# yahoo0742/COSNet

Measured on AMD Instinct MI355X. Metric: frame-pairs/sec (fwd+bwd) at 473x473 RGBD, higher is better.
Workload: dtype bf16; 1 GPU; RGBDSegmentation_RAA train step (fwd+loss+bwd+SGD), 473x473, batch 4 pairs/GPU; model=RGBDSegmentation_RAA(Bottleneck,[3,4,23,3],[3,4,6,3],1), global_batch=4, parallelism=dp1

## Files before the change

### cosnet_amd/csrc/gemm.hip

```cpp
#include "common.h"
#include "gemm.h"
#include "gemm_dev.h"
#include "../../include/cosnet_hip.h"

#include <type_traits>

namespace {

template <class T> struct Frag;
template <> struct Frag<bf16> { typedef bf16x8 type; };
template <> struct Frag<float> { typedef f32x4 type; };

__device__ __forceinline__ int mc_swz(int k, int granules_per_row) {
  int h = (k & 3) | (((k >> 3) & 1) << 2);
  return (granules_per_row >= 32 ? h : (h & 3)) << 2;
}

__device__ __forceinline__ int mc_swz8(int k) { return (k & 7) ^ ((k >> 5) & 1); }

__device__ __attribute__((aligned(16))) unsigned g_zero16[4];

__device__ __forceinline__ void glds16(const void* src, char* lds_wave_base) {
  __builtin_amdgcn_global_load_lds((const __attribute__((address_space(1))) void*)src,
                                   (__attribute__((address_space(3))) void*)lds_wave_base, 16, 0, 0);
// ... 726 lines not shown
          else if (p.wt)
            __builtin_amdgcn_raw_buffer_store_b128(pk, crs, (int)(((long long)(row - m0) * p.ldc + col) * 2), 0, 16);
          else
            *(u32x4*)dst = pk;
          if (smode) Chunk<bf16>::unpack(pk, v);
        } else {
          if (cmode == 2) {
            f32x4 q0 = *(const f32x4*)dst, q1 = *(const f32x4*)(dst + 4);
#pragma unroll
            for (int e = 0; e < 4; ++e) { v[e] += q0[e]; v[4 + e] += q1[e]; }
          }
          if (p.wt == 4) {
            __builtin_nontemporal_store(*(f32x4*)&v[0], (f32x4*)dst);
            __builtin_nontemporal_store(*(f32x4*)&v[4], (f32x4*)(dst + 4));
          } else if (p.wt) {
            const int off = (int)(((long long)(row - m0) * p.ldc + col) * 4);
            __builtin_amdgcn_raw_buffer_store_b128(__builtin_bit_cast(u32x4, *(f32x4*)&v[0]), crs, off, 0, 16);
            __builtin_amdgcn_raw_buffer_store_b128(__builtin_bit_cast(u32x4, *(f32x4*)&v[4]), crs, off + 16, 0, 16);
          } else {
            *(f32x4*)dst = *(f32x4*)&v[0];
            *(f32x4*)(dst + 4) = *(f32x4*)&v[4];
          }
        }
      } else {
#pragma unroll
        for (int e = 0; e < 8; ++e)
          if (col + e < p.N) {
            store_c<CT>(dst + e, v[e], cmode);
            v[e] = tof((CT)v[e]);
          }
      }
#ifndef CN_EPI_NOACC
      if constexpr (smode == 1) {
        const bool inA = row < segA_end;
#pragma unroll
        for (int e = 0; e < 8; ++e) {
          const float d = (col + e < p.N) ? v[e] - sk[e] : 0.f;
          if (inA) { sa1[e] += d; sa2[e] = fmaf(d, d, sa2[e]); }
          else { sb1[e] += d; sb2[e] = fmaf(d, d, sb2[e]); }
        }
      } else if constexpr (smode == 2) {
        float xv[8];
        if (full) {
          if constexpr (sizeof(CT) == 2) Chunk<bf16>::unpack(xpf[it], xv);
          else { *(u32x4*)&xv[0] = xpf[2 * it]; *(u32x4*)&xv[4] = xpf[2 * it + 1]; }
        } else {
          const CT* xs = (const CT*)p.br_x + (long long)row * p.br_ldx + col;
#pragma unroll
          for (int e = 0; e < 8; ++e) xv[e] = (col + e < p.N) ? tof(xs[e]) : 0.f;
        }
#pragma unroll
        for (int e = 0; e < 8; ++e) {
          float dd = (col + e < p.N && fmaf(xv[e], bk1[e], bsf[e]) > 0.f) ? v[e] : 0.f;
          sa1[e] += dd;
          sa2[e] = fmaf(dd, xv[e] - bmu[e], sa2[e]);
        }
      }
#endif
    }
    __syncthreads();
  }
#ifdef CN_EPI_NORED
  if constexpr (false) {
#else
  if constexpr (smode != 0) {
#endif
    constexpr int NW = NT / 64;
    const int nq = smode == 1 ? 4 : 2;
#pragma unroll
    for (int e = 0; e < 8; ++e) {
#pragma unroll
      for (int o = GPR; o < 64; o <<= 1) {
        sa1[e] += __shfl_xor(sa1[e], o, 64);
        sa2[e] += __shfl_xor(sa2[e], o, 64);
        if (smode == 1) {
          sb1[e] += __shfl_xor(sb1[e], o, 64);
          sb2[e] += __shfl_xor(sb2[e], o, 64);
        }
      }
    }
    float* red = cs;
    if (lane < GPR) {
#pragma unroll
      for (int e = 0; e < 8; ++e) {
        red[(wave * 4 + 0) * BN + c0t + e] = sa1[e];
        red[(wave * 4 + 1) * BN + c0t + e] = sa2[e];
        red[(wave * 4 + 2) * BN + c0t + e] = sb1[e];
        red[(wave * 4 + 3) * BN + c0t + e] = sb2[e];
      }
    }
    __syncthreads();
    float* ws = ((p.ngroup && p.grp.ST[batch]) ? p.grp.ST[batch] : p.st_ws) + (long long)tm * p.N;
    for (int t = tid; t < nq * BN; t += NT) {
      const int q = t / BN, c = t % BN;
      float a = 0.f;
#pragma unroll
      for (int w = 0; w < NW; ++w) a += red[(w * 4 + q) * BN + c];
      if (smode == 2 && q == 1 && n0 + c < p.N) a *= p.br_invstd[n0 + c];
      if (n0 + c < p.N) ws[(long long)(smode == 1 ? q + 1 : q) * p.st_plane + n0 + c] = a;
    }
    if (smode == 1 && tid < GPR) {
#pragma unroll
      for (int e = 0; e < 8; ++e)
        if (n0 + c0t + e < p.N) ws[n0 + c0t + e] = sk[e];
    }
  }
}

struct TileCfg { int bm, bn, wm, wn, s, pp; };
static constexpr TileCfg kCfg[] = {
    {128, 64, 2, 2, 2},
    {128, 128, 2, 2, 2},
    {128, 128, 2, 2, 3},
    {256, 128, 4, 2, 3},
    {128, 256, 2, 4, 3},
    {256, 256, 2, 4, 2},
    {128, 64, 2, 2, 4},
    {128, 128, 2, 2, 4},
    {256, 128, 4, 2, 2},
    {128, 256, 2, 4, 2},
    {256, 256, 4, 2, 2},
    {128, 128, 4, 2, 2},
    {128, 64, 4, 2, 2},
    {128, 128, 4, 2, 3},
    {128, 128, 4, 2, 4},
    {256, 128, 4, 2, 3},
    {128, 64, 4, 2, 4},
    {64, 128, 2, 4, 2},
    {256, 128, 4, 2, 3, 1},
    {128, 256, 2, 4, 3, 1},
    {256, 256, 2, 4, 2, 1},
};
constexpr int kNumCfg = sizeof(kCfg) / sizeof(kCfg[0]);
static int g_force_cfg = -1;

static long long cfg_blocks(int c, const GemmArgs& a, int batch) {
  return (long long)((a.M + kCfg[c].bm - 1) / kCfg[c].bm) * ((a.N + kCfg[c].bn - 1) / kCfg[c].bn) *
         batch * a.nsplit;
}

static long long tiles_of(int c, int M, int N) {
  return (long long)((M + kCfg[c].bm - 1) / kCfg[c].bm) * ((N + kCfg[c].bn - 1) / kCfg[c].bn);
}
static int heuristic_cfg(int M, int N, int K, int bz) {
  if (N <= 64) return 12;
  if (N >= 512 && K >= 2048 && tiles_of(10, M, N) * bz >= 200) return 20;
  if (tiles_of(11, M, N) * bz <= 256 && K >= 512) return 13;
  if (N >= 1024 && K <= 512 && tiles_of(10, M, N) * bz >= 200) return 10;
  return 11;
}

static int pick_cfg(const GemmArgs& a, int batch) {
  if (g_force_cfg >= 0 && g_force_cfg < kNumCfg) return g_force_cfg;
  if (a.cfg >= 0 && a.cfg < kNumCfg) return a.cfg;
  return heuristic_cfg(a.M, a.N, a.K, batch * a.nsplit);
}

template <class T, class CT, int C, int LA, int LB, int EPI = 0>
static int launch_c(const GemmArgs& a, int batch, hipStream_t st) {
  constexpr TileCfg c = kCfg[C];
  dim3 grid((a.M + c.bm - 1) / c.bm, (a.N + c.bn - 1) / c.bn, batch * a.nsplit);
  hipLaunchKernelGGL((gemm_kernel<T, CT, c.bm, c.bn, c.wm, c.wn, c.s, LA, LB, EPI, c.pp>), grid,
                     dim3(c.wm * c.wn * 64), 0, st, a);
  CN_CHECK_LAUNCH();
  return 0;
}

template <class T, int LA, int EPI>
static int launch_epi(const GemmArgs& a, int batch, hipStream_t st) {
  if constexpr (sizeof(T) == 4) {
    if (a.N <= 64 || cfg_blocks(1, a, batch) < 384) return launch_c<T, T, 0, LA, L_KC_DENSE, EPI>(a, batch, st);
    return launch_c<T, T, 1, LA, L_KC_DENSE, EPI>(a, batch, st);
  } else {
    switch (pick_cfg(a, batch)) {
      case 10: return launch_c<T, T, 10, LA, L_KC_DENSE, EPI>(a, batch, st);
      case 11: return launch_c<T, T, 11, LA, L_KC_DENSE, EPI>(a, batch, st);
      case 12: return launch_c<T, T, 12, LA, L_KC_DENSE, EPI>(a, batch, st);
      case 13: return launch_c<T, T, 13, LA, L_KC_DENSE, EPI>(a, batch, st);
      case 18: return launch_c<T, T, 18, LA, L_KC_DENSE, EPI>(a, batch, st);
      case 19: return launch_c<T, T, 19, LA, L_KC_DENSE, EPI>(a, batch, st);
      case 20: return launch_c<T, T, 20, LA, L_KC_DENSE, EPI>(a, batch, st);
      default: return CN_ERR_UNSUPPORTED;
    }
  }
}


template <class T, class CT, int LA, int LB>
static int launch_tile(const GemmArgs& a, int batch, hipStream_t st) {
  if constexpr (sizeof(T) == 2 && sizeof(CT) == 2 && (LA == L_KC_DENSE || LA == L_KC_CONV) &&
                LB == L_KC_DENSE) {
    if (a.c_mode == 2 && !a.row_map && !a.ngroup) {
      switch (pick_cfg(a, batch)) {
        case 10: return launch_c<T, CT, 10, LA, LB, 3>(a, batch, st);
        case 11: return launch_c<T, CT, 11, LA, LB, 3>(a, batch, st);
        case 12: return launch_c<T, CT, 12, LA, LB, 3>(a, batch, st);
        case 13: return launch_c<T, CT, 13, LA, LB, 3>(a, batch, st);
        case 20: return launch_c<T, CT, 20, LA, LB, 3>(a, batch, st);
        default: break;
      }
    }
  }
  if constexpr (sizeof(T) == 4) {
    if (a.N <= 64 || cfg_blocks(1, a, batch) < 384) return launch_c<T, CT, 0, LA, LB>(a, batch, st);
    return launch_c<T, CT, 1, LA, LB>(a, batch, st);
  } else {
    switch (pick_cfg(a, batch)) {
      case 0: return launch_c<T, CT, 0, LA, LB>(a, batch, st);
      case 1: return launch_c<T, CT, 1, LA, LB>(a, batch, st);
      case 2: return launch_c<T, CT, 2, LA, LB>(a, batch, st);
      case 3: return launch_c<T, CT, 3, LA, LB>(a, batch, st);
      case 4: return launch_c<T, CT, 4, LA, LB>(a, batch, st);
      case 5: return launch_c<T, CT, 5, LA, LB>(a, batch, st);
      case 6: return launch_c<T, CT, 6, LA, LB>(a, batch, st);
      case 7: return launch_c<T, CT, 7, LA, LB>(a, batch, st);
      case 8: return launch_c<T, CT, 8, LA, LB>(a, batch, st);
      case 9: return launch_c<T, CT, 9, LA, LB>(a, batch, st);
      case 10: return launch_c<T, CT, 10, LA, LB>(a, batch, st);
      case 11: return launch_c<T, CT, 11, LA, LB>(a, batch, st);
      case 13: return launch_c<T, CT, 13, LA, LB>(a, batch, st);
      case 14: return launch_c<T, CT, 14, LA, LB>(a, batch, st);
      case 15: return launch_c<T, CT, 15, LA, LB>(a, batch, st);
      case 16: return launch_c<T, CT, 16, LA, LB>(a, batch, st);
      case 17: return launch_c<T, CT, 17, LA, LB>(a, batch, st);
      case 18: case 19: case 20: {
        constexpr bool kc = LA != L_MC_DENSE && LA != L_MC_CONV && LB != L_MC_DENSE && LB != L_MC_CONV;
        if constexpr (kc) {
          const int c = pick_cfg(a, batch);
          if (c == 18) return launch_c<T, CT, 18, LA, LB>(a, batch, st);
          if (c == 19) return launch_c<T, CT, 19, LA, LB>(a, batch, st);
          return launch_c<T, CT, 20, LA, LB>(a, batch, st);
        } else {
          if (pick_cfg(a, batch) == 20) return launch_c<T, CT, 10, LA, LB>(a, batch, st);
          return launch_c<T, CT, 11, LA, LB>(a, batch, st);
        }
      }
      default: return launch_c<T, CT, 12, LA, LB>(a, batch, st);
    }
  }
}

template <class T, class CT>
static int launch_conv_g(const GemmArgs& a, int batch, hipStream_t st) {
  if constexpr (sizeof(T) == 4) {
    if (a.N <= 64 || cfg_blocks(1, a, batch) < 384) return launch_c<T, CT, 0, L_KC_CONV_G, L_KC_DENSE>(a, batch, st);
    return launch_c<T, CT, 1, L_KC_CONV_G, L_KC_DENSE>(a, batch, st);
  } else {
    const int c = pick_cfg(a, batch);
    if (c == 12) return launch_c<T, CT, 12, L_KC_CONV_G, L_KC_DENSE>(a, batch, st);
    if (c == 13) return launch_c<T, CT, 13, L_KC_CONV_G, L_KC_DENSE>(a, batch, st);
    return launch_c<T, CT, 11, L_KC_CONV_G, L_KC_DENSE>(a, batch, st);
  }
}

template <class T, class CT>
static int launch_kinds(const GemmArgs& a, int la, int lb, int batch, hipStream_t st) {
#define CN_CASE(A_, B_) \
  if (la == A_ && lb == B_) return launch_tile<T, CT, A_, B_>(a, batch, st);
  if (la == L_KC_CONV_G && lb == L_KC_DENSE) return launch_conv_g<T, CT>(a, batch, st);
  CN_CASE(L_KC_DENSE, L_KC_DENSE)
  CN_CASE(L_KC_CONV, L_KC_DENSE)
  CN_CASE(L_KC_DENSE, L_MC_DENSE)
  CN_CASE(L_MC_DENSE, L_MC_DENSE)
  CN_CASE(L_MC_DENSE, L_MC_CONV)
#undef CN_CASE
  return -10;
}

template <class CT, int LA, class T8 = f8e4m3>
static int launch_f8(const GemmArgs& a, int batch, hipStream_t st) {
  const int c = pick_cfg(a, batch);
  if constexpr (sizeof(CT) == 2 && std::is_same<T8, f8e4m3>::value) {
    if (a.st_mode == 1) {
      if (c == 12) return launch_c<T8, CT, 12, LA, L_KC_DENSE, 1>(a, batch, st);
      if (c == 13) return launch_c<T8, CT, 13, LA, L_KC_DENSE, 1>(a, batch, st);
      return launch_c<T8, CT, 11, LA, L_KC_DENSE, 1>(a, batch, st);
    }
  }
  if (a.st_mode) return CN_ERR_UNSUPPORTED;
  if (c == 12) return launch_c<T8, CT, 12, LA, L_KC_DENSE>(a, batch, st);
  if (c == 13) return launch_c<T8, CT, 13, LA, L_KC_DENSE>(a, batch, st);
  return launch_c<T8, CT, 11, LA, L_KC_DENSE>(a, batch, st);
}

template <int LB>
static int launch_f8_mc(const GemmArgs& a, int batch, hipStream_t st) {
  if (a.cfg == 13) return launch_c<f8e5m2, float, 13, L_MC_DENSE, LB>(a, batch, st);
  return launch_c<f8e5m2, float, 11, L_MC_DENSE, LB>(a, batch, st);
}

static bool buf_ok(int kind, const GemmArgs& a, bool is_a, int esz) {
  const long long ld = is_a ? a.lda : a.ldb;
  const ConvGeom& g = is_a ? a.ga : a.gb;
  const long long kspan = a.nsplit > 1 ? a.k_chunk : a.K;
  if (kind == L_KC_DENSE) return 256 * ld * esz < 0x80000000ll && (long long)a.K * esz < 0xFFFF0000ll;
  if (kind == L_KC_CONV) return (long long)g.N * g.H * g.W * ld * esz < 0x80000000ll;
  if (kind == L_MC_DENSE) return (kspan + 128) * ld * esz < 0xFFFF0000ll && 128 * ld * esz < 0x80000000ll;
  return true;
}

static int g_ws_mode = 1;
static size_t g_ws_launches = 0;
static bool ws_heuristic(const GemmArgs& a) {
  return a.K <= 256 && a.N >= 4 * a.K && a.M >= 8192;
}
static bool ws_eligible(const GemmArgs& a, int dtype, int c_f32, int la, int lb, int batch) {
  if (!g_ws_mode || g_force_cfg >= 0 || a.cfg >= 0) return false;
  if (dtype != DT_BF16 || c_f32 || la != L_KC_DENSE || lb != L_KC_DENSE) return false;
  if (batch != 1 || a.nsplit != 1 || a.row_map || a.ngroup || a.st_mode) return false;
  if ((a.c_mode != 0 && a.c_mode != 2) || a.bias || a.alpha != 1.f || a.scale_a || a.scale_b) return false;
  if (!cn_gemm_ws_supports(a)) return false;
  return g_ws_mode >= 2 || ws_heuristic(a);
}

int cn_gemm_dispatch(const GemmArgs& a_in, int dtype, int c_f32, int la, int lb, int batch, hipStream_t st) {
  GemmArgs a = a_in;
  a.wt = a.c_mode != 1 && a.c_mode != 3 ? 4 : 0;
  if (a.M <= 0 || a.N <= 0 || batch <= 0) return 0;
  const int esz = (dtype == DT_FP8 || dtype == DT_FP8_E5M2) ? 1 : dtype == DT_BF16 ? 2 : 4;
  const int bk = 128 / esz;
  if (la == L_KC_CONV && (a.ga.C % bk != 0 || !buf_ok(L_KC_CONV, a, true, esz))) la = L_KC_CONV_G;
  if (!buf_ok(la, a, true, esz) || !buf_ok(lb, a, false, esz)) return CN_ERR_SHAPE;
  if (ws_eligible(a, dtype, c_f32, la, lb, batch)) {
    ++g_ws_launches;
    return cn_gemm_ws_launch(a, g_ws_mode == 3 ? 1 : 0, st);
  }
  if (dtype == DT_FP8) {
    if (lb != L_KC_DENSE || a.nsplit != 1) return CN_ERR_UNSUPPORTED;
    if (a.st_mode && (a.st_mode != 1 || batch != 1 || a.row_map || a.c_mode || c_f32)) return CN_ERR_UNSUPPORTED;
    if (la == L_KC_DENSE) return c_f32 ? launch_f8<float, L_KC_DENSE>(a, batch, st) : launch_f8<bf16, L_KC_DENSE>(a, batch, st);
    if (la == L_KC_CONV) return c_f32 ? launch_f8<float, L_KC_CONV>(a, batch, st) : launch_f8<bf16, L_KC_CONV>(a, batch, st);
    if (la == L_KC_CONV_G) return c_f32 ? launch_f8<float, L_KC_CONV_G>(a, batch, st) : launch_f8<bf16, L_KC_CONV_G>(a, batch, st);
    return CN_ERR_UNSUPPORTED;
  }
  if (dtype == DT_FP8_E5M2 && la == L_MC_DENSE) {
    if (!c_f32 || a.st_mode || a.row_map || a.c_mode == 1 || a.c_mode == 2) return CN_ERR_UNSUPPORTED;
    if (lb == L_MC_DENSE) return launch_f8_mc<L_MC_DENSE>(a, batch, st);
    if (lb == L_MC_CONV) return launch_f8_mc<L_MC_CONV>(a, batch, st);
    return CN_ERR_UNSUPPORTED;
  }
  if (dtype == DT_FP8_E5M2) {
    if (lb != L_KC_DENSE || a.st_mode || a.nsplit != 1 || c_f32) return CN_ERR_UNSUPPORTED;
    if (la == L_KC_DENSE) return launch_f8<bf16, L_KC_DENSE, f8e5m2>(a, batch, st);
    if (la == L_KC_CONV) return launch_f8<bf16, L_KC_CONV, f8e5m2>(a, batch, st);
    if (la == L_KC_CONV_G) return launch_f8<bf16, L_KC_CONV_G, f8e5m2>(a, batch, st);
    return CN_ERR_UNSUPPORTED;
  }
  if (a.st_mode) {
    if ((batch != 1 && !(a.ngroup == batch && a.st_mode == 1)) || a.nsplit != 1 || a.row_map || a.c_mode ||
        lb != L_KC_DENSE || (la != L_KC_DENSE && la != L_KC_CONV && la != L_KC_CONV_G))
      return CN_ERR_UNSUPPORTED;
#define CN_EPI(T_, M_) \
    return la == L_KC_DENSE ? launch_epi<T_, L_KC_DENSE, M_>(a, batch, st) : \
           la == L_KC_CONV ? launch_epi<T_, L_KC_CONV, M_>(a, batch, st) : launch_epi<T_, L_KC_CONV_G, M_>(a, batch, st)
    if (dtype == DT_BF16) {
      if (a.st_mode == 1) CN_EPI(bf16, 1); else CN_EPI(bf16, 2);
    } else {
      if (a.st_mode == 1) CN_EPI(float, 1); else CN_EPI(float, 2);
    }
#undef CN_EPI
  }
  if (dtype == DT_BF16) {
    return c_f32 ? launch_kinds<bf16, float>(a, la, lb, batch, st)
                 : launch_kinds<bf16, bf16>(a, la, lb, batch, st);
  } else if (dtype == DT_F32) {
    return launch_kinds<float, float>(a, la, lb, batch, st);
  }
  return -11;
}

int cn_gemm_bm(int dtype, int M, int N, int K, int cfg) {
  if (dtype != DT_BF16) return kCfg[1].bm;
  if (g_force_cfg >= 0 && g_force_cfg < kNumCfg) return kCfg[g_force_cfg].bm;
  if (cfg >= 0 && cfg < kNumCfg) return kCfg[cfg].bm;
  return kCfg[heuristic_cfg(M, N, K, 1)].bm;
}

int cn_gemm_pick(int M, int N, int K, int batch_splits) {
  if (g_force_cfg >= 0 && g_force_cfg < kNumCfg) return g_force_cfg;
  return heuristic_cfg(M, N, K, batch_splits);
}

long long cn_gemm_cfg_blocks(int cfg, int M, int N) {
  GemmArgs a = {};
  a.M = M; a.N = N; a.nsplit = 1;
  return cfg_blocks(cfg, a, 1);
}

extern "C" int cn_gemm_force_config(int cfg) {
  if (cfg >= kNumCfg) return -1;
  g_force_cfg = cfg;
  return kNumCfg;
}

extern "C" int cn_gemm_ws_mode(int mode) {
  if (mode < 0 || mode > 3) return -1;
  const int prev = g_ws_mode;
  g_ws_mode = mode;
  return prev;
}

extern "C" size_t cn_gemm_ws_launches(void) { return g_ws_launches; }

template <int G>
__global__ __launch_bounds__(256) void splitk_reduce_k(const float* __restrict__ ws, int nsplit,
                                                       long long slab, long long n4,
                                                       float* __restrict__ out, int accumulate) {
  constexpr int OPB = 256 / G;
  __shared__ f32x4 red[G][OPB];
  const int o = threadIdx.x % OPB, g = threadIdx.x / OPB;
  for (long long base = (long long)blockIdx.x * OPB; base < n4; base += (long long)gridDim.x * OPB) {
    const long long i = base + o;
    f32x4 a = {0.f, 0.f, 0.f, 0.f};
    if (i < n4) {
      int s = g;
      for (; s + 7 * G < nsplit; s += 8 * G) {
        f32x4 v[8];
#pragma unroll
        for (int u = 0; u < 8; ++u) v[u] = *(const f32x4*)(ws + (long long)(s + u * G) * slab + 4 * i);
#pragma unroll
        for (int u = 0; u < 8; ++u) a += v[u];
      }
      for (; s < nsplit; s += G) a += *(const f32x4*)(ws + (long long)s * slab + 4 * i);
    }
    if (G > 1) {
      red[g][o] = a;
      __syncthreads();
      if (g == 0) {
#pragma unroll
        for (int q = 1; q < G; ++q) a += red[q][o];
      }
      __syncthreads();
    }
    if (g == 0 && i < n4) {
      if (accumulate) a += ((const f32x4*)out)[i];
      ((f32x4*)out)[i] = a;
    }
  }
}

int cn_splitk_reduce_impl(const float* ws, int nsplit, long long slab, long long n, float* out,
                          int accumulate, hipStream_t st) {
  if (n % 4 || slab % 4) return -2;
  const long long n4 = n / 4;
  int G = 1;
  while (G < 16 && 2 * G <= nsplit && n4 * G < (512ll << 10)) G *= 2;
  const int opb = 256 / G;
  long long b = (n4 + opb - 1) / opb;
  if (b > 4096) b = 4096;
#define CN_RED(GG) \
  hipLaunchKernelGGL(splitk_reduce_k<GG>, dim3((unsigned)b), dim3(256), 0, st, ws, nsplit, slab, n4, out, accumulate)
  switch (G) {
    case 1: CN_RED(1); break;
    case 2: CN_RED(2); break;
    case 4: CN_RED(4); break;
    case 8: CN_RED(8); break;
    default: CN_RED(16); break;
  }
#undef CN_RED
  CN_CHECK_LAUNCH();
  return 0;
}
```

### cosnet_amd/csrc/gemm_ws.hip

```cpp
#include "common.h"
#include "gemm.h"
#include "gemm_dev.h"
#include "../../include/cosnet_hip.h"

#include <algorithm>
#include <cstdlib>
#include <type_traits>

namespace {

struct WsArgs {
  int M, N;
  const bf16* A; long long lda;
  const bf16* B; long long ldb;
  bf16* C; long long ldc;
  int nslices;
  int wpx;
  int wt;
};

__device__ __forceinline__ u32x4 load16_asm(const void* p) {
  u32x4 v;
  asm volatile("global_load_dwordx4 %0, %1, off" : "=&v"(v) : "v"(p) : "memory");
  return v;
}

template <int KEEP, bool TIE, int N>
__device__ __forceinline__ void wait_keep(u32x4 (&x)[N]) {
  static_assert(KEEP < 64, "vmcnt is 6 bits");
  asm volatile("s_waitcnt vmcnt(%0)" :: "n"(KEEP) : "memory");
  if constexpr (TIE) {
#pragma unroll
    for (int i = 0; i < N; ++i) asm volatile("" : "+v"(x[i]));
  }
}

template <int KT, int BM, int BN, int WM, int WN, bool MODE2, bool BREG>
__global__ __launch_bounds__(WM * WN * 64, 1) void gemm_ws_kernel(WsArgs p) {
  constexpr int NT = WM * WN * 64;
  constexpr int BBYTES = KT * BN * 128, ASTG = KT * BM * 128;
  constexpr int TM = BM / WM, TN = BN / WN;
  constexpr int RM = TM / 16, RN = TN / 16;
  constexpr int NCA = BM * 8 / NT, NCB = BN * 8 / NT;
  constexpr int RSTEP = NT / 8;
  constexpr int CSB = TM * TN * 4;
  constexpr int GPR = TN / 8, RPP = 64 / GPR, IT = TM / RPP;
  static_assert(NCA >= 1 && NCA * NT == BM * 8 && NCB * NT == BN * 8, "tiles fill whole chunk rounds");
  static_assert(RSTEP % 8 == 0, "a thread's chunks share row & 7");
  static_assert(IT >= 1 && IT * RPP == TM && (RN & (RN - 1)) == 0, "epilogue passes");
  static_assert(BBYTES + 2 * ASTG + WM * WN * CSB <= 160 * 1024, "LDS budget");
  __shared__ __attribute__((aligned(16))) char smem[BBYTES + 2 * ASTG + WM * WN * CSB];

  const int tid = threadIdx.x, lane = tid & 63;
  const int wave = __builtin_amdgcn_readfirstlane(tid >> 6);
  const int wm = wave / WN, wn = wave % WN;

  const int xcd = blockIdx.x & 7, j = blockIdx.x >> 3;
  const int slice = j % p.nslices;
  const int walker = xcd * p.wpx + j / p.nslices, nwalk = 8 * p.wpx;
  const int n0 = slice * BN;
  const int m16 = (p.M + 15) >> 4;
  const int r0 = (int)((long long)m16 * walker / nwalk) * 16;
  const int r1 = min(p.M, (int)((long long)m16 * (walker + 1) / nwalk) * 16);
  if (r0 >= r1) return;
  const int ntiles = (r1 - r0 + BM - 1) / BM;

  char* Bs = smem;
  char* As = smem + BBYTES;
  float* cs = (float*)(smem + BBYTES + 2 * ASTG + wave * CSB);
  const int wbase = __builtin_amdgcn_readfirstlane((tid & ~63) * 16);

  const int kcol = ((tid & 7) ^ ((tid >> 3) & 7)) * 8;
  const int rl0 = tid >> 3;

  {
    const __amdgpu_buffer_rsrc_t rb = buf_rsrc(p.B + (long long)n0 * p.ldb);
#pragma unroll
    for (int i = 0; i < NCB; ++i) {
      const int rl = rl0 + RSTEP * i;
      const unsigned voff = n0 + rl < p.N ? (unsigned)((rl * p.ldb + kcol) * 2) : BUF_OOB;
#pragma unroll
      for (int kt = 0; kt < KT; ++kt) blds16(rb, voff, kt * 128, Bs + kt * BN * 128 + wbase + i * NT * 16);
    }
  }
  auto issue_a = [&](int t, char* stg) {
    const int m0 = r0 + t * BM;
    const __amdgpu_buffer_rsrc_t ra = buf_rsrc(p.A + (long long)m0 * p.lda);
#pragma unroll
    for (int i = 0; i < NCA; ++i) {
      const int rl = rl0 + RSTEP * i;
      const unsigned voff = m0 + rl < r1 ? (unsigned)((rl * p.lda + kcol) * 2) : BUF_OOB;
#pragma unroll
      for (int kt = 0; kt < KT; ++kt) blds16(ra, voff, kt * 128, stg + kt * BM * 128 + wbase + i * NT * 16);
    }
  };
  const int erow = wm * TM + lane / GPR, ecol = n0 + wn * TN + (lane % GPR) * 8;
  const bool col_ok = ecol < p.N;
  u32x4 xnx[MODE2 ? IT : 1], xpf[MODE2 ? IT : 1];
  auto fetch_c = [&](int t) {
    const int m0 = r0 + t * BM;
#pragma unroll
    for (int it = 0; it < IT; ++it) {
      const int row = m0 + erow + it * RPP;
      const bf16* src = (row < r1 && col_ok) ? p.C + (long long)row * p.ldc + ecol : p.C;
      xnx[it] = load16_asm(src);
    }
  };
  issue_a(0, As);
  if constexpr (MODE2) fetch_c(0);
  wait_keep<0, MODE2>(xnx);
  raw_barrier();

  bf16x8 breg[BREG ? KT * 2 : 1][RN];
  if constexpr (BREG) {
#pragma unroll
    for (int kt = 0; kt < KT; ++kt)
#pragma unroll
      for (int pc = 0; pc < 2; ++pc)
#pragma unroll
        for (int jj = 0; jj < RN; ++jj)
          breg[kt * 2 + pc][jj] = read_frag_kc_bf16(Bs + kt * BN * 128, wn * TN + jj * 16, pc, lane);
  }

  auto epilogue = [&](int t, auto aux_c, const f32x4 (&acc)[RM][RN]) {
    constexpr int AUX = decltype(aux_c)::value;
    const int m0 = r0 + t * BM;
    const __amdgpu_buffer_rsrc_t rc = buf_rsrc(p.C + (long long)m0 * p.ldc);
    const int g = lane >> 4;
#pragma unroll
    for (int i = 0; i < RM; ++i)
#pragma unroll
      for (int jj = 0; jj < RN; ++jj)
#pragma unroll
        for (int r = 0; r < 4; ++r)
          cs[(i * 16 + 4 * g + r) * TN + (((jj ^ (g & (RN - 1))) << 4) | (lane & 15))] = acc[i][jj][r];
    asm volatile("s_waitcnt lgkmcnt(0)" ::: "memory");
#pragma unroll
    for (int it = 0; it < IT; ++it) {
      const int rr = lane / GPR + it * RPP;
      const int c0 = ((lane % GPR) * 8) ^ ((((rr >> 2) & 3) & (RN - 1)) << 4);
      float v[8];
      *(f32x4*)&v[0] = *(const f32x4*)&cs[rr * TN + c0];
      *(f32x4*)&v[4] = *(const f32x4*)&cs[rr * TN + c0 + 4];
      if constexpr (MODE2) {
        float q[8];
        Chunk<bf16>::unpack(xpf[it], q);
#pragma unroll
        for (int e = 0; e < 8; ++e) v[e] += q[e];
      }
      const int row = erow + it * RPP;
      const unsigned off = (m0 + row < r1 && col_ok) ? (unsigned)(((long long)row * p.ldc + ecol) * 2) : BUF_OOB;
      __builtin_amdgcn_raw_buffer_store_b128(Chunk<bf16>::pack(v), rc, (int)off, 0, AUX);
    }
    asm volatile("" ::: "memory");
  };

#pragma unroll 1
  for (int t = 0; t < ntiles; ++t) {
    char* cur = As + (t & 1) * ASTG;
    if constexpr (MODE2) {
#pragma unroll
      for (int it = 0; it < IT; ++it) xpf[it] = xnx[it];
    }
    if (t + 1 < ntiles) {
      issue_a(t + 1, As + ((t + 1) & 1) * ASTG);
      if constexpr (MODE2) fetch_c(t + 1);
    }
    f32x4 acc[RM][RN];
#pragma unroll
    for (int i = 0; i < RM; ++i)
#pragma unroll
      for (int jj = 0; jj < RN; ++jj) acc[i][jj] = (f32x4){0.f, 0.f, 0.f, 0.f};
#pragma unroll
    for (int kt = 0; kt < KT; ++kt)
#pragma unroll
      for (int pc = 0; pc < 2; ++pc) {
        bf16x8 af[RM], bfr[RN];
#pragma unroll
        for (int i = 0; i < RM; ++i) af[i] = read_frag_kc_bf16(cur + kt * BM * 128, wm * TM + i * 16, pc, lane);
#pragma unroll
        for (int jj = 0; jj < RN; ++jj) {
          if constexpr (BREG) bfr[jj] = breg[kt * 2 + pc][jj];
          else bfr[jj] = read_frag_kc_bf16(Bs + kt * BN * 128, wn * TN + jj * 16, pc, lane);
        }
#pragma unroll
        for (int i = 0; i < RM; ++i)
#pragma unroll
          for (int jj = 0; jj < RN; ++jj)
            acc[i][jj] = __builtin_amdgcn_mfma_f32_16x16x32_bf16(af[i], bfr[jj], acc[i][jj], 0, 0, 0);
      }
    if (p.wt == 4) epilogue(t, std::integral_constant<int, 2>{}, acc);
    else if (p.wt) epilogue(t, std::integral_constant<int, 16>{}, acc);
    else epilogue(t, std::integral_constant<int, 0>{}, acc);
    if (t + 1 < ntiles) {
      wait_keep<IT, MODE2>(xnx);
      raw_barrier();
    }
  }
}

template <int KT, int BM, int BN, int WM, int WN, bool BREG>
int launch_ws(const GemmArgs& a, int cus, int cap, hipStream_t st) {
  WsArgs w;
  w.M = a.M; w.N = a.N;
  w.A = (const bf16*)a.A; w.lda = a.lda;
  w.B = (const bf16*)a.B; w.ldb = a.ldb;
  w.C = (bf16*)a.C; w.ldc = a.ldc;
  w.nslices = (a.N + BN - 1) / BN;
  w.wt = a.wt;
  const int per_xcd = cus / 8;
  const int want = (int)((((long long)a.M + 15) / 16 + 7) / 8);
  w.wpx = std::min(per_xcd / w.nslices, std::max(want, 1));
  if (cap > 0) w.wpx = std::min(w.wpx, cap);
  if (w.wpx < 1) return CN_ERR_UNSUPPORTED;
  const dim3 grid(8 * w.wpx * w.nslices), block(WM * WN * 64);
  if (a.c_mode == 2)
    hipLaunchKernelGGL((gemm_ws_kernel<KT, BM, BN, WM, WN, true, BREG>), grid, block, 0, st, w);
  else
    hipLaunchKernelGGL((gemm_ws_kernel<KT, BM, BN, WM, WN, false, BREG>), grid, block, 0, st, w);
  CN_CHECK_LAUNCH();
  return 0;
}

int device_cus() {
  static const int n = [] {
    int dev = 0, v = 0;
    if (hipGetDevice(&dev) != hipSuccess) return 0;
    if (hipDeviceGetAttribute(&v, hipDeviceAttributeMultiprocessorCount, dev) != hipSuccess) return 0;
    return v;
  }();
  return n;
}

int ws_bn(int K) { return K == 512 ? 64 : 128; }

}

bool cn_gemm_ws_supports(const GemmArgs& a) {
  if (a.K != 64 && a.K != 128 && a.K != 256 && a.K != 512) return false;
  if (a.ka_lim < a.K || a.kb_lim < a.K) return false;
  if (a.N % 8 || a.ldc % 8 || (uintptr_t)a.C % 16) return false;
  if (a.lda % 8 || a.ldb % 8 || (uintptr_t)a.A % 16 || (uintptr_t)a.B % 16) return false;
  if (256 * a.ldc * 2 >= 0x80000000ll) return false;
  const int cus = device_cus();
  return cus >= 8 && (a.N + ws_bn(a.K) - 1) / ws_bn(a.K) <= cus / 8;
}

int cn_gemm_ws_launch(const GemmArgs& a, int walkers_per_xcd, hipStream_t st) {
  const int cus = device_cus();
  switch (a.K) {
    case 64:
      if (a.c_mode == 2) return launch_ws<1, 64, 128, 2, 2, true>(a, cus, walkers_per_xcd, st);
      return launch_ws<1, 128, 128, 4, 2, true>(a, cus, walkers_per_xcd, st);
    case 128: return launch_ws<2, 128, 128, 4, 2, true>(a, cus, walkers_per_xcd, st);
    case 256: return launch_ws<4, 64, 128, 2, 4, true>(a, cus, walkers_per_xcd, st);
    case 512: return launch_ws<8, 32, 64, 2, 2, false>(a, cus, walkers_per_xcd, st);
    default: return CN_ERR_UNSUPPORTED;
  }
}
```

Baseline: 136.6 frame-pairs/s.

## Add ring-buffered weight-stationary GEMM kernel for K=512/1024 and enable heuristic

Adds a new weight-stationary walker GEMM kernel that keeps B in registers and streams A through a multi-stage LDS ring of K-chunks, so loads for the next chunk or tile overlap the MFMA work on the current one. It replaces the K=512 path with this kernel, adds K=1024 support, and widens the heuristic so K=512 GEMMs with large M are routed to the walker path. Holding the full B slice in registers raises register pressure, and the larger BN narrows which shapes qualify for the walker path.

```diff
diff --git a/cosnet_amd/csrc/gemm.hip b/cosnet_amd/csrc/gemm.hip
--- a/cosnet_amd/csrc/gemm.hip
+++ b/cosnet_amd/csrc/gemm.hip
@@ -1052,7 +1052,7 @@
 static int g_ws_mode = 1;
 static size_t g_ws_launches = 0;
 static bool ws_heuristic(const GemmArgs& a) {
-  return a.K <= 256 && a.N >= 4 * a.K && a.M >= 8192;
+  return a.K <= 512 && a.N >= 4 * a.K && a.M >= 8192;
 }
 static bool ws_eligible(const GemmArgs& a, int dtype, int c_f32, int la, int lb, int batch) {
   if (!g_ws_mode || g_force_cfg >= 0 || a.cfg >= 0) return false;
diff --git a/cosnet_amd/csrc/gemm_ws.hip b/cosnet_amd/csrc/gemm_ws.hip
--- a/cosnet_amd/csrc/gemm_ws.hip
+++ b/cosnet_amd/csrc/gemm_ws.hip
@@ -6,6 +6,7 @@
 #include <algorithm>
 #include <cstdlib>
 #include <type_traits>
+#include <utility>
 
 namespace {
 
@@ -199,8 +200,175 @@
   }
 }
 
-template <int KT, int BM, int BN, int WM, int WN, bool BREG>
-int launch_ws(const GemmArgs& a, int cus, int cap, hipStream_t st) {
+constexpr int ring_tile_ends(int ch, int ns, int nch) {
+  int n = 0;
+  for (int d = 0; d <= ns - 2; ++d) n += ((ch - d) % nch + nch) % nch == nch - 1;
+  return n;
+}
+
+template <int... I, class Fn>
+__device__ __forceinline__ void static_for(std::integer_sequence<int, I...>, Fn&& f) {
+  (f(std::integral_constant<int, I>{}), ...);
+}
+
+template <int KT, int CK, int NS, int BM, int BN, int WM, int WN, bool MODE2>
+__global__ __launch_bounds__(WM * WN * 64, 1) void gemm_ws_ring_kernel(WsArgs p) {
+  constexpr int NT = WM * WN * 64;
+  constexpr int NCH = KT / CK, STG = CK * BM * 128;
+  constexpr int TM = BM / WM, TN = BN / WN;
+  constexpr int RM = TM / 16, RN = TN / 16;
+  constexpr int NCA = BM * 8 / NT, RSTEP = NT / 8;
+  constexpr int CSB = TM * TN * 4;
+  constexpr int GPR = TN / 8, RPP = 64 / GPR, IT = TM / RPP;
+  constexpr int F = NCA * CK;
+  constexpr int E = IT + (MODE2 ? IT : 0);
+  static_assert(NCH * CK == KT && NCH >= 2 && (NCH & (NCH - 1)) == 0, "whole chunks");
+  static_assert(NS >= 3 && (NS & (NS - 1)) == 0, "ring depth");
+  static_assert(NCA >= 1 && NCA * NT == BM * 8 && RSTEP % 8 == 0, "tiles fill whole chunk rounds");
+  static_assert(IT >= 1 && IT * RPP == TM && (RN & (RN - 1)) == 0, "epilogue passes");
+  static_assert(NS * STG + WM * WN * CSB <= 160 * 1024, "LDS budget");
+  __shared__ __attribute__((aligned(16))) char smem[NS * STG + WM * WN * CSB];
+
+  const int tid = threadIdx.x, lane = tid & 63;
+  const int wave = __builtin_amdgcn_readfirstlane(tid >> 6);
+  const int wm = wave / WN, wn = wave % WN;
+
+  const int xcd = blockIdx.x & 7, j = blockIdx.x >> 3;
+  const int slice = j % p.nslices;
+  const int walker = xcd * p.wpx + j / p.nslices, nwalk = 8 * p.wpx;
+  const int n0 = slice * BN;
+  const int m16 = (p.M + 15) >> 4;
+  const int r0 = (int)((long long)m16 * walker / nwalk) * 16;
+  const int r1 = min(p.M, (int)((long long)m16 * (walker + 1) / nwalk) * 16);
+  if (r0 >= r1) return;
+  const int ntiles = (r1 - r0 + BM - 1) / BM;
+
+  char* As = smem;
+  float* cs = (float*)(smem + NS * STG + wave * CSB);
+  const int wbase = __builtin_amdgcn_readfirstlane((tid & ~63) * 16);
+  const int kcol = ((tid & 7) ^ ((tid >> 3) & 7)) * 8;
+  const int rl0 = tid >> 3;
+
+  bf16x8 breg[KT * 2][RN];
+#pragma unroll
+  for (int jj = 0; jj < RN; ++jj) {
+    const int col = min(n0 + wn * TN + jj * 16 + (lane & 15), p.N - 1);
+    const bf16* src = p.B + (long long)col * p.ldb + (lane >> 4) * 8;
+#pragma unroll
+    for (int q = 0; q < KT * 2; ++q) breg[q][jj] = *(const bf16x8*)(src + q * 32);
+  }
+  asm volatile("" ::: "memory");
+
+  auto issue_a = [&](int t, int ch) {
+    const int m0 = r0 + t * BM;
+    const __amdgpu_buffer_rsrc_t ra = buf_rsrc(p.A + (long long)m0 * p.lda + ch * (CK * 64));
+    char* stg = As + ((t * NCH + ch) & (NS - 1)) * STG;
+#pragma unroll
+    for (int i = 0; i < NCA; ++i) {
+      const int rl = rl0 + RSTEP * i;
+      const unsigned voff = m0 + rl < r1 ? (unsigned)((rl * p.lda + kcol) * 2) : BUF_OOB;
+#pragma unroll
+      for (int kt = 0; kt < CK; ++kt) blds16(ra, voff, kt * 128, stg + kt * BM * 128 + wbase + i * NT * 16);
+    }
+  };
+  const int erow = wm * TM + lane / GPR, ecol = n0 + wn * TN + (lane % GPR) * 8;
+  const bool col_ok = ecol < p.N;
+  u32x4 xc[MODE2 ? IT : 1];
+  auto fetch_c = [&](int t) {
+    const int m0 = r0 + t * BM;
+#pragma unroll
+    for (int it = 0; it < IT; ++it) {
+      const int row = m0 + erow + it * RPP;
+      const bf16* src = (row < r1 && col_ok) ? p.C + (long long)row * p.ldc + ecol : p.C;
+      xc[it] = load16_asm(src);
+    }
+  };
+  static_for(std::make_integer_sequence<int, NS - 1>{}, [&](auto cc) {
+    constexpr int c = decltype(cc)::value;
+    issue_a(c / NCH, c % NCH);
+  });
+  if constexpr (MODE2) fetch_c(0);
+  wait_keep<0, MODE2>(xc);
+#pragma unroll
+  for (int q = 0; q < KT * 2; ++q)
+#pragma unroll
+    for (int jj = 0; jj < RN; ++jj) asm volatile("" : "+v"(breg[q][jj]));
+  raw_barrier();
+
+  auto epilogue = [&](int t, auto aux_c, const f32x4 (&acc)[RM][RN]) {
+    constexpr int AUX = decltype(aux_c)::value;
+    const int m0 = r0 + t * BM;
+    const __amdgpu_buffer_rsrc_t rc = buf_rsrc(p.C + (long long)m0 * p.ldc);
+    const int g = lane >> 4;
+#pragma unroll
+    for (int i = 0; i < RM; ++i)
+#pragma unroll
+      for (int jj = 0; jj < RN; ++jj)
+#pragma unroll
+        for (int r = 0; r < 4; ++r)
+          cs[(i * 16 + 4 * g + r) * TN + (((jj ^ (g & (RN - 1))) << 4) | (lane & 15))] = acc[i][jj][r];
+    asm volatile("s_waitcnt lgkmcnt(0)" ::: "memory");
+#pragma unroll
+    for (int it = 0; it < IT; ++it) {
+      const int rr = lane / GPR + it * RPP;
+      const int c0 = ((lane % GPR) * 8) ^ ((((rr >> 2) & 3) & (RN - 1)) << 4);
+      float v[8];
+      *(f32x4*)&v[0] = *(const f32x4*)&cs[rr * TN + c0];
+      *(f32x4*)&v[4] = *(const f32x4*)&cs[rr * TN + c0 + 4];
+      if constexpr (MODE2) {
+        float q[8];
+        Chunk<bf16>::unpack(xc[it], q);
+#pragma unroll
+        for (int e = 0; e < 8; ++e) v[e] += q[e];
+      }
+      const int row = erow + it * RPP;
+      const unsigned off = (m0 + row < r1 && col_ok) ? (unsigned)(((long long)row * p.ldc + ecol) * 2) : BUF_OOB;
+      __builtin_amdgcn_raw_buffer_store_b128(Chunk<bf16>::pack(v), rc, (int)off, 0, AUX);
+    }
+    asm volatile("" ::: "memory");
+  };
+
+#pragma unroll 1
+  for (int t = 0; t < ntiles; ++t) {
+    f32x4 acc[RM][RN];
+#pragma unroll
+    for (int i = 0; i < RM; ++i)
+#pragma unroll
+      for (int jj = 0; jj < RN; ++jj) acc[i][jj] = (f32x4){0.f, 0.f, 0.f, 0.f};
+    static_for(std::make_integer_sequence<int, NCH>{}, [&](auto chc) {
+      constexpr int ch = decltype(chc)::value;
+      issue_a(t + (ch + NS - 1) / NCH, (ch + NS - 1) % NCH);
+      const char* cur = As + ((t * NCH + ch) & (NS - 1)) * STG;
+#pragma unroll
+      for (int kt = 0; kt < CK; ++kt)
+#pragma unroll
+        for (int pc = 0; pc < 2; ++pc) {
+          bf16x8 af[RM];
+#pragma unroll
+          for (int i = 0; i < RM; ++i) af[i] = read_frag_kc_bf16(cur + kt * BM * 128, wm * TM + i * 16, pc, lane);
+#pragma unroll
+          for (int i = 0; i < RM; ++i)
+#pragma unroll
+            for (int jj = 0; jj < RN; ++jj)
+              acc[i][jj] = __builtin_amdgcn_mfma_f32_16x16x32_bf16(af[i], breg[(ch * CK + kt) * 2 + pc][jj],
+                                                                   acc[i][jj], 0, 0, 0);
+        }
+      if constexpr (ch == NCH - 1) {
+        if constexpr (MODE2) wait_keep<NCH * F, true>(xc);
+        if (p.wt == 4) epilogue(t, std::integral_constant<int, 2>{}, acc);
+        else if (p.wt) epilogue(t, std::integral_constant<int, 16>{}, acc);
+        else epilogue(t, std::integral_constant<int, 0>{}, acc);
+        if constexpr (MODE2) fetch_c(t + 1);
+      }
+      wait_keep<(NS - 2) * F + ring_tile_ends(ch, NS, NCH) * E, false>(xc);
+      raw_barrier();
+    });
+  }
+  asm volatile("s_waitcnt vmcnt(0)" ::: "memory");
+}
+
+template <class Kern>
+int launch_walkers(Kern kern, int BN, int NT, const GemmArgs& a, int cus, int cap, hipStream_t st) {
   WsArgs w;
   w.M = a.M; w.N = a.N;
   w.A = (const bf16*)a.A; w.lda = a.lda;
@@ -213,13 +381,24 @@
   w.wpx = std::min(per_xcd / w.nslices, std::max(want, 1));
   if (cap > 0) w.wpx = std::min(w.wpx, cap);
   if (w.wpx < 1) return CN_ERR_UNSUPPORTED;
-  const dim3 grid(8 * w.wpx * w.nslices), block(WM * WN * 64);
-  if (a.c_mode == 2)
-    hipLaunchKernelGGL((gemm_ws_kernel<KT, BM, BN, WM, WN, true, BREG>), grid, block, 0, st, w);
-  else
-    hipLaunchKernelGGL((gemm_ws_kernel<KT, BM, BN, WM, WN, false, BREG>), grid, block, 0, st, w);
+  const dim3 grid(8 * w.wpx * w.nslices), block(NT);
+  hipLaunchKernelGGL(kern, grid, block, 0, st, w);
   CN_CHECK_LAUNCH();
   return 0;
+}
+
+template <int KT, int CK, int NS, int BM, int BN, int WM, int WN>
+int launch_ring(const GemmArgs& a, int cus, int cap, hipStream_t st) {
+  if (a.c_mode == 2)
+    return launch_walkers(gemm_ws_ring_kernel<KT, CK, NS, BM, BN, WM, WN, true>, BN, WM * WN * 64, a, cus, cap, st);
+  return launch_walkers(gemm_ws_ring_kernel<KT, CK, NS, BM, BN, WM, WN, false>, BN, WM * WN * 64, a, cus, cap, st);
+}
+
+template <int KT, int BM, int BN, int WM, int WN, bool BREG>
+int launch_ws(const GemmArgs& a, int cus, int cap, hipStream_t st) {
+  if (a.c_mode == 2)
+    return launch_walkers(gemm_ws_kernel<KT, BM, BN, WM, WN, true, BREG>, BN, WM * WN * 64, a, cus, cap, st);
+  return launch_walkers(gemm_ws_kernel<KT, BM, BN, WM, WN, false, BREG>, BN, WM * WN * 64, a, cus, cap, st);
 }
 
 int device_cus() {
@@ -232,18 +411,18 @@
   return n;
 }
 
-int ws_bn(int K) { return K == 512 ? 64 : 128; }
+constexpr int WS_BN = 128;
 
 }
 
 bool cn_gemm_ws_supports(const GemmArgs& a) {
-  if (a.K != 64 && a.K != 128 && a.K != 256 && a.K != 512) return false;
+  if (a.K != 64 && a.K != 128 && a.K != 256 && a.K != 512 && a.K != 1024) return false;
   if (a.ka_lim < a.K || a.kb_lim < a.K) return false;
   if (a.N % 8 || a.ldc % 8 || (uintptr_t)a.C % 16) return false;
   if (a.lda % 8 || a.ldb % 8 || (uintptr_t)a.A % 16 || (uintptr_t)a.B % 16) return false;
   if (256 * a.ldc * 2 >= 0x80000000ll) return false;
   const int cus = device_cus();
-  return cus >= 8 && (a.N + ws_bn(a.K) - 1) / ws_bn(a.K) <= cus / 8;
+  return cus >= 8 && (a.N + WS_BN - 1) / WS_BN <= cus / 8;
 }
 
 int cn_gemm_ws_launch(const GemmArgs& a, int walkers_per_xcd, hipStream_t st) {
@@ -254,7 +433,8 @@
       return launch_ws<1, 128, 128, 4, 2, true>(a, cus, walkers_per_xcd, st);
     case 128: return launch_ws<2, 128, 128, 4, 2, true>(a, cus, walkers_per_xcd, st);
     case 256: return launch_ws<4, 64, 128, 2, 4, true>(a, cus, walkers_per_xcd, st);
-    case 512: return launch_ws<8, 32, 64, 2, 2, false>(a, cus, walkers_per_xcd, st);
+    case 512: return launch_ring<8, 4, 4, 64, 128, 2, 4>(a, cus, walkers_per_xcd, st);
+    case 1024: return launch_ring<16, 4, 4, 64, 128, 1, 8>(a, cus, walkers_per_xcd, st);
     default: return CN_ERR_UNSUPPORTED;
   }
 }
```

New measurement: 137.6 frame-pairs/s (median of 6 runs). No clear change (+0.8%).
